# fmbnicola/P3D-RayTracer

Measured on AMD Instinct MI355X. Metric: Mrays/s (primary+secondary), higher is better.
Workload: dtype f32; 1 GPU; balls_low.p3f 1024x1024, Whitted MAX_DEPTH=4, BVH, no AA (BASELINE configs[1]); rays_per_frame=4944908, stack_mode=literal, outputs_per_rank=float RGB + hit ID (16 B/px) + u8 image (3 B/px), all written to HBM, tile_order=cost, frames_in_flight=6, streams=2 bulk (pass 1) + 2 tail (hand-off launches), parallelism=image rows in 8-row stripes, round-robin over 1 GPU(s)

## Files before the change

### p3d-raytracer_amd/__init__.py

```python
import ctypes as C
import os
import subprocess

import numpy as np

HERE = os.path.dirname(os.path.abspath(__file__))
LIB_PATH = os.environ.get("P3D_LIB") or os.path.join(HERE, "libp3d.so")

ACCEL_NONE, ACCEL_GRID, ACCEL_BVH = 0, 1, 2
WHITTED, PATHTRACE = 0, 1
TILE_ORDER_COST, TILE_ORDER_FRAME = 0, 1
STACK_LITERAL, STACK_PER_PIXEL = 0, 1
CHAIN_AUTO, CHAIN_MEGAKERNEL, CHAIN_PER_LEVEL = 0, 1, 2
SAMPLE_JITTER, SAMPLE_TENT = 0, 1
LOAD_LEGACY_F11 = 1
DEBUG_NONE, DEBUG_TEST_INTERSECT, DEBUG_DEPTH_MAP = 0, 1, 2
HANDOFF_COMPACT, HANDOFF_DENSE = 0, 1
UPDATE_REFIT, UPDATE_REBUILD = 0, 1

EXPORTS = [
    "p3d_abi_version", "p3d_last_error", "p3d_device_count", "p3d_config_default",
    "p3d_scene_create", "p3d_scene_create_device_bvh", "p3d_scene_destroy", "p3d_scene_set_skybox", "p3d_render_tile", "p3d_render_tile_device",
    "p3d_scene_status", "p3d_scene_set_tail_stream", "p3d_scene_join", "p3d_object_intercepts", "p3d_object_normal", "p3d_skybox_color",
    "p3d_trace_closest", "p3d_trace_any", "p3d_host_scene_load", "p3d_host_scene_destroy",
# ... 624 lines not shown
                out = acc.render(min(samples_per_pass, acc.total - acc.samples_done), want_rgb8=want_rgb8, stats=stats)
                yield acc.samples_done, out
        finally:
            acc.close()

    def adaptive(self, cfg, rel_error, min_samples=16, tile=None, reserved=(0, 0)):
        return AdaptiveAccumulator(self, cfg, tile or self.full_tile(), rel_error, min_samples, reserved)

    def render_adaptive(self, cfg, samples_per_pass, rel_error, min_samples=16, tile=None, want_rgb8=False, stats=True):
        if samples_per_pass < 1:
            raise ValueError("samples_per_pass must be at least 1")
        ad = self.adaptive(cfg, rel_error, min_samples, tile)
        try:
            while ad.samples_done < ad.total:
                out = ad.render(min(samples_per_pass, ad.total - ad.samples_done), want_rgb8=want_rgb8, stats=stats)
                active = ad.active_pixels
                yield ad.samples_done, active, out
                if active == 0:
                    break
        finally:
            ad.close()

    def status(self):
        return int(self._L.p3d_scene_status(self._h))

    def set_tail_stream(self, stream=None):
        raw = getattr(stream, "cuda_stream", stream)
        _check(self._L.p3d_scene_set_tail_stream(self._h, C.c_void_p(raw) if raw else None))

    def join(self, stream=None, host_wait=False):
        raw = getattr(stream, "cuda_stream", stream)
        _check(self._L.p3d_scene_join(self._h, C.c_void_p(raw) if raw else None, 1 if host_wait else 0))

    def debug_limits(self, trip_bound=0, max_rounds=0, halo_chain=0, leftover_pool=0):
        lim = (C.c_uint32 * 4)(trip_bound, max_rounds, halo_chain, leftover_pool)
        _check(self._L.p3d_debug_scene_limits(self._h, C.cast(lim, C.c_void_p)))

    def render_features(self, cfg, samples=0, tile=None):
        t = tile or self.full_tile()
        nd = np.zeros((t.h, t.w, 4), np.float32)
        ac = np.zeros((t.h, t.w, 4), np.float32)
        _check(self._L.p3d_render_features(self._h, C.byref(cfg), C.byref(t), int(samples), nd.ctypes.data, ac.ctypes.data))
        return nd, ac

    def render_features_device(self, cfg, d_normal_depth, d_albedo_cov, samples=0, tile=None, stream=0):
        raw = getattr(stream, "cuda_stream", stream)
        _check(self._L.p3d_render_features_device(self._h, C.byref(cfg), C.byref(tile or self.full_tile()), int(samples),
                                                  C.c_void_p(d_normal_depth or None), C.c_void_p(d_albedo_cov or None),
                                                  C.c_void_p(raw or None)))

    def render_device(self, cfg, tile, d_rgb=0, d_hit=0, d_rgb8=0, stream=0, stats=None):
        _check(self._L.p3d_render_tile_device(self._h, C.byref(cfg), C.byref(tile), C.c_void_p(d_rgb or None),
                                              C.c_void_p(d_hit or None), C.c_void_p(d_rgb8 or None),
                                              C.c_void_p(stream or None), C.byref(stats) if stats is not None else None))

    def trace_closest(self, accel, origin, direction, want_t=False):
        o = np.ascontiguousarray(origin, np.float32)
        d = np.ascontiguousarray(direction, np.float32)
        n = o.shape[0]
        hit = np.zeros(n, np.int32)
        hp = np.zeros((n, 3), np.float32)
        t = np.zeros(n, np.float32) if want_t else None
        _check(self._L.p3d_trace_closest(self._h, int(accel), n, o.ctypes.data, d.ctypes.data, hit.ctypes.data,
                                         t.ctypes.data if want_t else None, hp.ctypes.data))
        return (hit, hp, t) if want_t else (hit, hp)

    def object_intercepts(self, obj, origin, direction):
        o = np.ascontiguousarray(origin, np.float32)
# ... 336 lines not shown
```

### p3d-raytracer_amd/csrc/capi_common.hpp

```cpp
#pragma once
#include <hip/hip_runtime.h>

#include <algorithm>
#include <cmath>
#include <cstdio>
#include <cstdlib>
#include <cstring>
#include <memory>
#include <string>
#include <type_traits>
#include <vector>

#include "../host/p3d_error.hpp"
#include "kernels.hpp"
#include "lbvh.hpp"
#include "grid_build.hpp"
#include "xform_prims.hpp"
#include "p3d.h"
#include "p3d_debug.h"
#include "wavefront.hpp"
#include "queries.hpp"
#include "pt_kernel.hpp"
#include "adaptive.hpp"
#include "features.hpp"
// ... 46 lines not shown
struct SchedEntry {
  uint32_t accel = 0, aa = 0, spp = 0, pt = 0, tiles_x = 0, tiles_y = 0;
  int32_t max_depth = 0, x0 = 0, y0 = 0, w = 0, h = 0, stripe_h = 0, stripe_stride = 0;
  Scratch cost, sched;
  hipEvent_t ready = nullptr;
  hipStream_t built_on = nullptr;
  uint64_t last_use = 0;
  bool built = false;
  bool same_key(const SchedEntry& o) const {
    return accel == o.accel && aa == o.aa && spp == o.spp && pt == o.pt && tiles_x == o.tiles_x && tiles_y == o.tiles_y && max_depth == o.max_depth && x0 == o.x0 && y0 == o.y0 &&
           w == o.w && h == o.h && stripe_h == o.stripe_h && stripe_stride == o.stripe_stride;
  }
};

}

struct p3d_scene {
  int device = 0;
  std::vector<SchedEntry> sched;
  uint64_t sched_clock = 0;
  float4* d_blob = nullptr;
  uint32_t blob_f4 = 0;
  uint32_t off_nodes = 0, off_bgeom = 0, off_ogeom = 0, off_normals = 0, off_mats = 0, off_lights = 0;
  uint32_t* d_cell_start = nullptr;
  uint32_t* d_cell_items = nullptr;
  uint32_t* d_emitters = nullptr;
  uint32_t* d_sky[6] = {nullptr, nullptr, nullptr, nullptr, nullptr, nullptr};
  bool has_sky = false;
  DevScene dev{};
  bool has_bvh = false, has_grid = false;
  uint32_t bvh_max_depth = 0;
  float device_bvh_ms = 0;
  Scratch levels, spill, deferred, wf_rays, wf_keys, wf_sorted, wf_final, out_rgb, out_hit, out_rgb8, q_in, q_out;
  Scratch ho_where, ho_entries, ho_meta, ho_first, ho_first_sample, ho_touched, ho_lists, ho_check, ho_counters, ho_row_chain, ho_halo_pix, ho_ucount;
  std::vector<int64_t> ho_chain_key;
  bool has_spheres = false;
  uint32_t* d_halo_verdict = nullptr;
  float root_min[3] = {0, 0, 0}, root_max[3] = {0, 0, 0};
  bool zero_weight_reflections = false;
  unsigned long long* d_stats = nullptr;
  uint32_t* d_status = nullptr;
  uint32_t last_status = 0;
  p3d_debug_limits dbg{0, 0, 0, 0};
  hipEvent_t ev0 = nullptr, ev1 = nullptr, ev_mid = nullptr, ev_p1 = nullptr;
  hipStream_t tail_stream = nullptr;
  hipEvent_t ev_tail_go = nullptr, ev_tail_done = nullptr;
  bool tail_pending = false;
  uint64_t cam_gen = 0;
  bool device_bvh = false;
  uint64_t geom_gen = 0;
  std::vector<uint32_t> obj_tm;
  std::vector<float4> create_boxes;
  lbvh::Workspace lbvh_ws;
  bool lbvh_topology = false;
  Scratch upd_stage;
  std::vector<lbvh::UpdateRecord> upd_host;
  Scratch rest;
  Scratch xf_stage;
  std::vector<uint4> xf_host;
  bool uploaded_grid = false;
  uint64_t cell_start_cap = 0, cell_items_cap = 0;
  uint32_t grid_items = 0;
  grid_build::Workspace grid_ws;
};

namespace {

void drop_schedules(p3d_scene* s) {
  for (SchedEntry& e : s->sched)
    if (e.ready) (void)hipEventDestroy(e.ready);
  s->sched.clear();
}

bool camera_usable(const p3d_camera& c) {
  const float f[17] = {c.eye[0], c.eye[1], c.eye[2], c.u[0], c.u[1], c.u[2], c.v[0], c.v[1], c.v[2], c.n[0], c.n[1], c.n[2],
                       c.plane_dist, c.w, c.h, c.focal_ratio, c.aperture};
// ... 46 lines not shown
```

### p3d-raytracer_amd/csrc/capi_debug.hpp

```cpp
#pragma once
#include "capi_common.hpp"

extern "C" {

int p3d_debug_scene_limits(p3d_scene* s, const p3d_debug_limits* limits) {
  static const bool enabled = [] { const char* e = getenv("P3D_TEST_HOOKS"); return e && e[0] == '1' && e[1] == 0; }();
  if (!enabled) return fail(P3D_ERR_UNSUPPORTED, "p3d_debug_scene_limits: test hooks are off (start the process with P3D_TEST_HOOKS=1)");
  if (!s) return fail(P3D_ERR_INVALID, "p3d_debug_scene_limits: null scene");
  s->dbg = limits ? *limits : p3d_debug_limits{0, 0, 0, 0};
  return P3D_OK;
}

#ifdef P3D_PT_PROFILE
int p3d_debug_set_pt_prof(void* device_ptr) {
  unsigned long long* p = static_cast<unsigned long long*>(device_ptr);
  return hipMemcpyToSymbol(HIP_SYMBOL(p3d::g_pt_prof), &p, sizeof(p)) == hipSuccess ? P3D_OK : P3D_ERR_NO_DEVICE;
}
#endif
#ifdef P3D_TIMELINE
int p3d_debug_set_timeline(void* device_ptr) {
  unsigned long long* p = static_cast<unsigned long long*>(device_ptr);
  return hipMemcpyToSymbol(HIP_SYMBOL(p3d::g_timeline), &p, sizeof(p)) == hipSuccess ? P3D_OK : P3D_ERR_NO_DEVICE;
}
int p3d_debug_copy_sched(p3d_scene* s, uint32_t* host_sched, size_t n_sched, uint32_t* host_cost, size_t n_cost) {
  if (s->sched.empty()) return P3D_ERR_INVALID;
  (void)hipDeviceSynchronize();
  if (hipMemcpy(host_sched, s->sched[0].sched.p, n_sched * 4, hipMemcpyDeviceToHost) != hipSuccess) return P3D_ERR_NO_DEVICE;
  return hipMemcpy(host_cost, s->sched[0].cost.p, n_cost * 4, hipMemcpyDeviceToHost) == hipSuccess ? P3D_OK : P3D_ERR_NO_DEVICE;
}
#endif

}
```

### p3d-raytracer_amd/csrc/capi_frame.hpp

```cpp
#pragma once
#include "capi_frame_plan.hpp"

namespace {

constexpr uint32_t kWfHistWords = kWfBins + 32;
#ifndef P3D_REDO_LANES
#define P3D_REDO_LANES 64
#endif
inline uint32_t redo_lanes() {
  static const uint32_t v = [] {
    const char* e = getenv("P3D_REDO_LANES");
    const int n = e ? atoi(e) : P3D_REDO_LANES;
    return (uint32_t)(n >= 1 && n <= 64 ? n : P3D_REDO_LANES);
  }();
  return v;
}
inline uint32_t round1_lanes() {
  static const uint32_t v = [] {
    const char* e = getenv("P3D_ROUND1_LANES");
    const int n = e ? atoi(e) : 64;
    return (uint32_t)(n >= 1 && n <= 64 ? n : 64);
  }();
  return v;
}
// ... 315 lines not shown
    uint64_t pool_entries = H.dense ? (uint64_t)2 * H.cap * H.n_units : s->dbg.leftover_pool ? s->dbg.leftover_pool : std::max<uint64_t>(1u << 16, (uint64_t)kPoolEntriesPerUnit * H.n_units);
    if (!H.dense) pool_entries = std::min<uint64_t>(pool_entries, (uint64_t)2 * H.cap * H.n_units);
    if (pool_entries > 0xffffffffull) return fail(P3D_ERR_CAPACITY, "hit_stack hand-off records exceed 2^32 entries: render the frame in smaller tiles or use P3D_STACK_PER_PIXEL");
    H.pool_cap = (uint32_t)pool_entries;
    if (int rc = s->ho_entries.ensure((size_t)pool_entries * sizeof(uint2))) return rc;
    if (!H.dense)
      if (int rc = s->ho_where.ensure((size_t)2 * H.n_units * sizeof(uint32_t))) return rc;
    if (int rc = s->ho_meta.ensure((size_t)2 * H.n_units * 4)) return rc;
    if (int rc = s->ho_first.ensure((size_t)H.n_units * sizeof(float4))) return rc;
    if (int rc = s->ho_first_sample.ensure(cfg->antialiasing ? (size_t)H.n_units * 4 : 16)) return rc;
    touched_bytes = ((size_t)H.n_units / 32 + 2) * 4;
    if (int rc = s->ho_touched.ensure(touched_bytes)) return rc;
    if (int rc = s->ho_lists.ensure((size_t)4 * H.n_units * sizeof(uint4))) return rc;
    if (!H.dense && !lds_scene)
      if (int rc = s->ho_check.ensure((size_t)H.n_units * sizeof(uint32_t))) return rc;
    counter_words = 32 + (per_level ? ((uint32_t)cfg->max_depth + 1) * (kWfSegments * kWfCounterStride + kWfHistWords) : 0);
    if (int rc = s->ho_counters.ensure((size_t)counter_words * sizeof(uint32_t))) return rc;
    if (per_level) {
      wf_seg_cap = H.n_units / 4 + 4096;
      if (int rc = s->wf_rays.ensure((size_t)kWfSegments * wf_seg_cap * 2 * sizeof(float4))) return rc;
      if (int rc = s->wf_keys.ensure((size_t)kWfSegments * wf_seg_cap * sizeof(uint32_t))) return rc;
      if (int rc = s->wf_sorted.ensure((size_t)H.n_units * 2 * sizeof(float4))) return rc;
      if (int rc = s->wf_final.ensure((size_t)H.n_units * sizeof(float4))) return rc;
    }
    H.entries = (uint2*)s->ho_entries.p;
    H.where = (uint32_t*)s->ho_where.p;
    H.meta = (uint32_t*)s->ho_meta.p;
    H.meta0 = H.meta + H.n_units;
    H.first = (float4*)s->ho_first.p;
    H.first_sample = (uint32_t*)s->ho_first_sample.p;
    H.touched = (uint32_t*)s->ho_touched.p;
    H.row_chain = nullptr;
    H.halo_pix = nullptr;
    if (any_chain) {
      if (int rc = s->ho_row_chain.ensure((size_t)tile->h)) return rc;
      if (int rc = s->ho_halo_pix.ensure((size_t)tile->h * kHaloChain * 4)) return rc;
      H.row_chain = (const uint8_t*)s->ho_row_chain.p;
      H.halo_pix = (const uint32_t*)s->ho_halo_pix.p;
    }
    if (literal && want_counts) {
      if (int rc = s->ho_ucount.ensure((size_t)(kNumStats + kCh0Counters) * H.n_units * sizeof(uint32_t))) return rc;
      H.ucount = (uint32_t*)s->ho_ucount.p;
      H.uch0 = H.ucount + (size_t)kNumStats * H.n_units;
    }
    H.list_cap = H.n_units;
    H.count = want_counts ? 1u : 0u;
    H.max_rounds = std::min<uint32_t>(H.n_units + 2, 4096);
    if (s->dbg.max_rounds) H.max_rounds = s->dbg.max_rounds;
    for (int i = 0; i < 4; ++i) ho_list[i] = (uint4*)s->ho_lists.p + (size_t)i * H.n_units;
    ho_counters = (uint32_t*)s->ho_counters.p;
    H.counters = ho_counters;
    H.pool_top = ho_counters + kHoPoolTop;
    H.check_list = (H.dense || lds_scene) ? nullptr : (uint32_t*)s->ho_check.p;
    H.check_n = ho_counters + kHoCheckN;
    return P3D_OK;
  }

  int halo_memo() {
    const Handoff& H = P.hand;
    if (!plan.literal || !H.halo) return P3D_OK;
    const DevCamera& cam = s->dev.cam;
    halo_blocks = (H.rows * kHaloChain + kBlock - 1) / kBlock;
    const uint32_t max_chain = s->dbg.halo_chain ? std::min<uint32_t>(s->dbg.halo_chain, kHaloChain) : kHaloChain;
    const std::vector<int64_t> key = {tile->x0, tile->y0, tile->w, tile->h, tile->stripe_h, tile->stripe_stride, cam.res_x, cam.res_y,
                                      cfg->antialiasing ? 1 : 0, cfg->antialiasing ? (int64_t)cfg->spp_sqrt : 1, (int64_t)cfg->seed,
                                      cfg->sample_mode, cfg->depth_of_field, cfg->sample_disk, max_chain, (int64_t)(intptr_t)st};
// ... 355 lines not shown
```

### p3d-raytracer_amd/csrc/capi_frame_plan.hpp

```cpp
#pragma once
#include "capi_common.hpp"

namespace {

#ifndef P3D_PT_SUB4_MIN_SPP_SQRT
#define P3D_PT_SUB4_MIN_SPP_SQRT 4
#endif
#ifndef P3D_WHITTED_SUB4_MIN_SPP_SQRT
#define P3D_WHITTED_SUB4_MIN_SPP_SQRT 2
#endif
constexpr uint32_t kWhittedSub4MinSppSqrt = P3D_WHITTED_SUB4_MIN_SPP_SQRT;
constexpr uint32_t kPtSub4MinSppSqrt = P3D_PT_SUB4_MIN_SPP_SQRT;
constexpr uint32_t kLdsSceneLimitBytesPt = 16 * 1024;
constexpr uint32_t kLdsSceneLimitBytes = 26 * 1024;
static_assert(kLdsSceneLimitBytes / 32 < 4096 && kLdsSceneLimitBytesPt / 32 < 4096, "the 6-byte stack entries of LDS-staged scenes keep 12 index bits (device_core.hpp Stack)");
constexpr size_t kLaunchScratchBudget = (size_t)4 << 30;
constexpr uint32_t kMaxLaunchThreads = 1u << 24;

void tile_shape(uint64_t pixels, uint32_t& w, uint32_t& h) {
  static const int forced = [] { const char* e = getenv("P3D_TILE_SHAPE"); return e ? atoi(e) : 0; }();
  int shape = forced;
  if (shape != 88 && shape != 84 && shape != 44) shape = 88;
  w = shape == 44 ? 4 : 8;
  h = shape == 88 ? 8 : 4;
// ... 5 lines not shown
  uint32_t bvh_max_depth, n_lights;
  bool zero_weight_reflections;
};
inline SceneFacts scene_facts(const p3d_scene* s) {
  return SceneFacts{s->off_nodes, s->off_ogeom, s->blob_f4, s->bvh_max_depth, s->dev.n_lights, s->zero_weight_reflections};
}

uint32_t stack_bound(const SceneFacts& s, uint32_t accel, bool whitted) {
  if (accel != P3D_ACCEL_BVH) return 1;
  const uint32_t per = s.bvh_max_depth > 1 ? s.bvh_max_depth - 1 : 1;
  return whitted ? (s.n_lights + 1) * per : per;
}

enum FrameMode { kFrame, kAdaptivePass, kFeatures };

struct FramePlan {
  FrameMode mode;
  bool pt, literal;
  uint32_t bound;
  uint32_t stage_lo, stage_hi;
  bool lds_scene, lds_spill;
  uint32_t window, cap, spill_entries;
  int stack_mode;
  bool sub4, cold_lds;
  uint32_t tpw, tph;
  size_t lds_bytes;
  uint32_t levels, deferred;
  bool per_level;
  int sh, ss;
  uint32_t tiles_x, total_bands, bands_per_launch, xcd_chunk;
  uint32_t halo_blocks_max, adapt_blocks, feat_blocks, max_threads;
  size_t levels_bytes, spill_bytes, deferred_bytes;
  bool sched_ok, repair_tiles;

  uint32_t blocks_for(uint32_t ntiles) const {
    const uint32_t groups = (ntiles + 8 * xcd_chunk - 1) / (8 * xcd_chunk);
    return groups * 8 * xcd_chunk;
  }
};

int plan_frame(const SceneFacts& s, const p3d_config* cfg, const p3d_tile* tile, uint32_t sample_begin, uint32_t sample_end, FrameMode mode,
               uint32_t resident, FramePlan& plan) {
  const bool feat = mode == kFeatures, adapt = mode == kAdaptivePass;
  const uint32_t chain_launch = feat ? (uint32_t)P3D_CHAIN_AUTO : cfg->chain_launch;
  const int sh = tile->stripe_h > 0 ? tile->stripe_h : 1, ss = tile->stripe_h > 0 ? tile->stripe_stride : 1;
  const bool pt = cfg->integrator == P3D_PATHTRACE && cfg->antialiasing;
  const bool literal = !feat && cfg->stack_mode == P3D_STACK_LITERAL && !pt && cfg->accel == P3D_ACCEL_BVH;
  const uint32_t bound = stack_bound(s, cfg->accel, !pt);
  const uint32_t stage_lo = s.off_nodes, stage_hi = (cfg->accel == P3D_ACCEL_BVH && !pt) ? s.off_ogeom : s.blob_f4;
  const size_t stage_bytes = (size_t)(stage_hi - stage_lo) * sizeof(float4);
  const bool lds_scene = stage_bytes <= (pt ? kLdsSceneLimitBytesPt : kLdsSceneLimitBytes) && (bound <= 24 || !pt);
  const bool lds_spill = lds_scene && !pt && (bound > 24 || stage_bytes + (size_t)stack_lds_f4(false, bound) * sizeof(float4) > 20 * 1024);
  uint32_t window = 8;
  if (const char* e = getenv("P3D_LDS_STACK_ENTRIES")) {
    window = 1;
    while (window < (uint32_t)std::max(1, atoi(e)) && window < 1024) window *= 2;
  }
  const bool spilling = cfg->accel == P3D_ACCEL_BVH && !(lds_scene && !lds_spill);
  const uint32_t cap = cfg->accel == P3D_ACCEL_BVH ? (spilling ? window : bound) : 1;
  const uint32_t spill_entries = (spilling && bound > cap) ? bound : 0;
  const uint32_t lds_scene_f4 = lds_scene ? stage_hi - stage_lo : 0;
  const uint32_t launch_samples = sample_end - sample_begin;
  const bool sub4 = !feat && ((pt && launch_samples >= kPtSub4MinSppSqrt * kPtSub4MinSppSqrt) ||
                              (!pt && !literal && !lds_scene && cfg->antialiasing && launch_samples >= kWhittedSub4MinSppSqrt * kWhittedSub4MinSppSqrt));
  const bool cold_lds = !pt && !lds_scene && !cfg->antialiasing;
  uint32_t tpw = sub4 ? 4 : 8, tph = sub4 ? 4 : 8;
// ... 16 lines not shown
  const uint32_t total_bands = ((uint32_t)tile->h + tp - 1) / tp;
  if (tile->stripe_h > 0 && sh % (int)tp == 0 && bands_per_launch >= (uint32_t)sh / tp)
    bands_per_launch = (bands_per_launch / ((uint32_t)sh / tp)) * ((uint32_t)sh / tp);
  bands_per_launch = std::min(bands_per_launch, total_bands);
  if (per_level && bands_per_launch < total_bands) {
    if (chain_launch == P3D_CHAIN_PER_LEVEL) return fail(P3D_ERR_CAPACITY, "chain_launch = PER_LEVEL: tile too large for one launch");
    per_level = false;
    scratch_per_thread += (size_t)levels * sizeof(float4);
    const uint32_t lt = (uint32_t)std::min<size_t>(kMaxLaunchThreads, kLaunchScratchBudget / std::max<size_t>(scratch_per_thread, 1));
    bands_per_launch = std::min(std::max<uint32_t>(1, lt / (tiles_x * kBlock)), total_bands);
    if (tile->stripe_h > 0 && sh % (int)tp == 0 && bands_per_launch >= (uint32_t)sh / tp)
      bands_per_launch = (bands_per_launch / ((uint32_t)sh / tp)) * ((uint32_t)sh / tp);
  }
  plan.mode = mode; plan.pt = pt; plan.literal = literal; plan.bound = bound; plan.stage_lo = stage_lo; plan.stage_hi = stage_hi;
  plan.lds_scene = lds_scene; plan.lds_spill = lds_spill; plan.window = window; plan.cap = cap; plan.spill_entries = spill_entries;
  plan.stack_mode = stack_mode; plan.sub4 = sub4; plan.cold_lds = cold_lds; plan.tpw = tpw; plan.tph = tph; plan.lds_bytes = lds_bytes;
  plan.levels = levels; plan.deferred = deferred; plan.per_level = per_level; plan.sh = sh; plan.ss = ss;
  plan.tiles_x = tiles_x; plan.total_bands = total_bands; plan.bands_per_launch = bands_per_launch;
  plan.xcd_chunk = lds_scene ? 1u : tiles_x;
  plan.sched_ok = cfg->tile_order == P3D_TILE_ORDER_COST && cfg->max_depth > 0;
  const uint32_t halo_blocks_max = plan.halo_blocks_max = literal ? ((uint32_t)tile->h * kHaloChain + kBlock - 1) / kBlock : 0;
  const uint32_t adapt_blocks = plan.adapt_blocks = adapt ? std::max<uint32_t>(1, std::min<uint32_t>(resident, (uint32_t)(((size_t)tile->w * tile->h + (sub4 ? 15 : 63)) / (sub4 ? 16 : 64)))) : 0;
  const uint32_t feat_blocks = plan.feat_blocks = feat ? plan.blocks_for(tiles_x * total_bands) : 0;
  if (feat && (uint64_t)feat_blocks * kBlock * std::max<uint32_t>(spill_entries, 1) > 0xffffffffull)
    return fail(P3D_ERR_CAPACITY, "p3d_render_features: tile too large for one launch over a tree this deep (split the tile)");
  const uint32_t max_threads = plan.max_threads = adapt ? adapt_blocks * kBlock : (feat ? feat_blocks * kBlock : (plan.blocks_for(tiles_x * bands_per_launch) + halo_blocks_max) * kBlock);
  const size_t tile_units = (size_t)tile->h * ((size_t)tile->w + kHaloChain);
  const size_t level_cols = per_level ? std::max<size_t>(tile_units, literal ? (size_t)max_threads : 0) : (size_t)max_threads;
  plan.levels_bytes = std::max<size_t>(16, (size_t)levels * level_cols * sizeof(float4));
  const size_t halo_backing = literal && s.bvh_max_depth > 8 ? (size_t)s.bvh_max_depth * tile->h * kBlock * sizeof(uint2) : 0;
  plan.spill_bytes = std::max<size_t>(16, std::max((size_t)spill_entries * max_threads * sizeof(uint2), halo_backing));
  plan.deferred_bytes = std::max<size_t>(16, (size_t)deferred * max_threads * sizeof(float4));
  plan.repair_tiles = literal && lds_scene && !per_level;
  return P3D_OK;
}

}
```

### p3d-raytracer_amd/csrc/handoff.hpp

```cpp
#pragma once

#include <cstdint>

#include <hip/hip_runtime.h>

namespace p3d {

constexpr uint32_t kHaloChain = 16;
constexpr uint32_t kMetaTouched = 1u << 17;
constexpr uint32_t kNoUnit = 0xffffffffu;

enum HandoffCounter { kHoChecked = 0, kHoRedone, kHoRounds, kHoPoolTop, kHoListA, kHoListB, kHoListC, kHoListD, kHoCheckN, kHoRound0, kHoRound1, kHoNumCounters };
constexpr uint32_t kHoErrLeftoverCap = 1u;
constexpr uint32_t kHoErrNoFixedPoint = 2u;
constexpr uint32_t kHoErrTrips = 4u;
constexpr uint32_t kHoErrList = 8u;
constexpr uint32_t kHoErrHalo = 16u;

struct Handoff {
  uint32_t n_units;
  uint32_t row_units;
  uint32_t halo;
  uint32_t rows;
  uint32_t cap;
  uint32_t persistent;
  uint32_t list_cap;
  uint32_t max_rounds;
  uint32_t round_base;
  uint32_t count;
  uint32_t lanes;
  uint2* entries;
  uint32_t* where;
  uint32_t* pool_top;
  uint32_t* check_list;
  uint32_t* check_n;
  uint32_t pool_cap;
  uint32_t dense;
  uint32_t* meta;
  uint32_t* meta0;
  float4* first;
  uint32_t* first_sample;
  uint32_t* touched;
  const uint8_t* row_chain;
  const uint32_t* halo_pix;
  uint4* list_in;
  uint4* list_out;
  uint32_t* n_in;
  uint32_t* n_out;
  uint32_t* counters;
  uint32_t* ucount;
  uint32_t* uch0;
};
constexpr int kCh0Counters = 5;

__host__ __device__ inline int find_prev_bit(const uint32_t* bits, uint32_t lo, uint32_t i) {
  if (i <= lo) return -1;
  uint32_t w = (i - 1) >> 5;
  const uint32_t wlo = lo >> 5;
  uint32_t word = bits[w] & (0xffffffffu >> (31u - ((i - 1) & 31u)));
  while (true) {
    if (w == wlo) word &= 0xffffffffu << (lo & 31u);
    if (word) return (int)(w * 32u + 31u - (uint32_t)__builtin_clz(word));
    if (w == wlo) return -1;
    --w;
    word = bits[w];
  }
}
__host__ __device__ inline int find_next_bit(const uint32_t* bits, uint32_t i, uint32_t hi) {
  if (i >= hi) return -1;
  uint32_t w = i >> 5;
  const uint32_t whi = (hi - 1) >> 5;
  uint32_t word = bits[w] & (0xffffffffu << (i & 31u));
  while (true) {
    if (w == whi) word &= 0xffffffffu >> (31u - ((hi - 1) & 31u));
    if (word) return (int)(w * 32u + (uint32_t)__builtin_ffs((int)word) - 1u);
    if (w == whi) return -1;
    ++w;
    word = bits[w];
  }
}

__host__ __device__ inline int handoff_pred(const Handoff& H, uint32_t u) {
  if (!H.row_chain) return find_prev_bit(H.touched, 0, u);
  uint32_t row = u / H.row_units, i = u;
  while (true) {
    const uint32_t lo = row * H.row_units;
    const int b = find_prev_bit(H.touched, lo, i);
    if (b >= 0) return b;
    if (H.row_chain[row] || row == 0) return -1;
    i = lo;
    --row;
  }
}
__host__ __device__ inline int handoff_succ(const Handoff& H, uint32_t u) {
  if (!H.row_chain) return find_next_bit(H.touched, u + 1, H.n_units);
  uint32_t row = u / H.row_units, i = u + 1;
  while (true) {
    const uint32_t hi = (row + 1) * H.row_units;
    const int b = find_next_bit(H.touched, i, hi);
    if (b >= 0) return b;
    ++row;
    if (row >= H.rows || H.row_chain[row]) return -1;
    i = hi;
  }
}

__device__ __forceinline__ uint32_t leftover_at(const Handoff& H, uint32_t slot, uint32_t unit) {
  return H.dense ? (slot * H.n_units + unit) * H.cap : H.where[slot * H.n_units + unit];
}
__device__ __forceinline__ uint32_t leftover_alloc(const Handoff& H, uint32_t n, uint32_t slot, uint32_t unit, uint32_t* status, bool announce) {
  if (H.dense) return (slot * H.n_units + unit) * H.cap;
  const uint32_t lane = threadIdx.x & 63u;
  if (announce && H.check_list) {
    const unsigned long long m = __ballot(n != 0);
    uint32_t first = 0;
    if (lane == 63 && m) first = atomicAdd(H.check_n, (uint32_t)__popcll(m));
    first = __shfl(first, 63, 64);
    if (n != 0) H.check_list[first + (uint32_t)__popcll(m & ((1ull << lane) - 1ull))] = unit;
  }
  uint32_t incl = n;
  for (int o = 1; o < 64; o <<= 1) {
    const uint32_t v = __shfl_up(incl, o, 64);
    if ((int)lane >= o) incl += v;
  }
  const uint32_t total = __shfl(incl, 63, 64);
  uint32_t base = 0;
  if (lane == 63 && total) base = atomicAdd(H.pool_top, total);
  base = __shfl(base, 63, 64);
  const uint32_t at = base + incl - n;
  if (n == 0) return kNoUnit;
  if ((unsigned long long)at + n > H.pool_cap) {
    atomicOr(status, kHoErrLeftoverCap);
    return kNoUnit;
  }
  H.where[slot * H.n_units + unit] = at;
  return at;
}

__device__ __forceinline__ bool handoff_touched(const Handoff& H, uint32_t u) { return (H.touched[u >> 5] >> (u & 31u)) & 1u; }
// ... 9 lines not shown
```

### p3d-raytracer_amd/csrc/handoff_kernels.hpp

```cpp

namespace p3d {

struct UnitPlace {
  int c, r, x, y;
  bool halo;
  bool valid;
};
__device__ __forceinline__ UnitPlace no_place() { return UnitPlace{0, 0, 0, 0, false, false}; }
template <class T>
__device__ __forceinline__ T stripe_row(T y0, int r, int sh, int ss) { return y0 + (T)(r / sh) * sh * ss + (r % sh); }
__device__ __forceinline__ int image_row(const RenderParams& P, int r) {
  return stripe_row<int>(P.y0, r, P.stripe_h > 0 ? P.stripe_h : 1, P.stripe_h > 0 ? P.stripe_stride : 1);
}
__device__ __forceinline__ UnitPlace place_of_unit(const RenderParams& P, uint32_t unit) {
  const Handoff& H = P.hand;
  UnitPlace u;
  const uint32_t row = unit / H.row_units, j = unit - row * H.row_units;
  u.r = (int)row - P.row0;
  u.halo = j < H.halo;
  u.valid = true;
  if (u.halo) {
    const uint32_t fp = H.halo_pix[row * H.halo + j];
    u.valid = fp != kNoUnit;
    u.c = 0;
// ... 11 lines not shown
  const uint32_t slot = (blockIdx.x - P.tile_blocks) * kBlock + lane;
  const uint32_t row = slot / kHaloChain, j = slot % kHaloChain;
  if (H.halo == 0 || row >= H.rows || !H.row_chain[row]) return false;
  unit = row * H.row_units + j;
  return H.halo_pix[row * H.halo + j] != kNoUnit;
}
__device__ __forceinline__ bool tile_pixel(const RenderParams& P, uint32_t tx, uint32_t ty, uint32_t tws, uint32_t ths, uint32_t px, int& c, int& r) {
  c = (int)((tx << tws) + (px & ((1u << tws) - 1u)));
  r = (int)((ty << ths) + (px >> tws));
  return px < (1u << (tws + ths)) && c < P.w && r < P.h;
}
__device__ __forceinline__ uint32_t unit_of_pixel(const RenderParams& P, int c, int r) {
  return (uint32_t)(P.row0 + r) * P.hand.row_units + P.hand.halo + (uint32_t)c;
}
__device__ __forceinline__ bool unit_of_lane(const RenderParams& P, bool halo_block, uint32_t tx, uint32_t ty, uint32_t tws, uint32_t ths,
                                             uint32_t lane, uint32_t& unit) {
  if (halo_block) return halo_unit_of_lane(P, lane, unit);
  int c, r;
  const bool in = tile_pixel(P, tx, ty, tws, ths, lane, c, r);
  unit = unit_of_pixel(P, c, r);
  return in;
}
__device__ __forceinline__ uint32_t list_count(const uint32_t* n, uint32_t cap) {
  const uint32_t v = __hip_atomic_load(n, __ATOMIC_RELAXED, __HIP_MEMORY_SCOPE_AGENT);
  return v > cap ? cap : v;
}
__device__ __forceinline__ uint4 list_entry(const uint4* list, uint32_t i) {
  const uint32_t* e = reinterpret_cast<const uint32_t*>(list + i);
  return make_uint4(__hip_atomic_load(e, __ATOMIC_RELAXED, __HIP_MEMORY_SCOPE_AGENT), __hip_atomic_load(e + 1, __ATOMIC_RELAXED, __HIP_MEMORY_SCOPE_AGENT),
                    __hip_atomic_load(e + 2, __ATOMIC_RELAXED, __HIP_MEMORY_SCOPE_AGENT), __hip_atomic_load(e + 3, __ATOMIC_RELAXED, __HIP_MEMORY_SCOPE_AGENT));
}

template <bool SPILL, class CT>
__device__ __forceinline__ void seed_stack(Stack& st, const Handoff& H, uint32_t pred, uint32_t slot_count, CT& ct) {
  stack_clear(st);
  const uint32_t n = slot_count & 0xffffu, slot = slot_count >> 16;
  const uint32_t at = n ? leftover_at(H, slot, pred) : 0u;
  for (uint32_t e = 0; e < n; ++e) {
    const uint2 v = H.entries[at + e];
    push<SPILL>(st, v.x, __uint_as_float(v.y), ct);
  }
}
template <bool STATS>
__device__ __forceinline__ void store_unit_counters(const Handoff& H, uint32_t unit, const Counters<STATS>& ct, const uint32_t* ch0,
                                                    unsigned long long* stats) {
  if (!STATS) return;
  for (int s = 0; s < kNumStats; ++s)
    if (s != kMaxStack) H.ucount[(size_t)s * H.n_units + unit] = ct.get(s);
  for (int k = 0; k < kCh0Counters; ++k) H.uch0[(size_t)k * H.n_units + unit] = ch0[k];
  atomicMax(&stats[kMaxStack], (unsigned long long)ct.get(kMaxStack));
}
template <bool STATS>
__device__ __forceinline__ void replace_ch0_counters(const Handoff& H, uint32_t unit, const Counters<STATS>& cc, unsigned long long* stats) {
  if (!STATS) return;
  for (int k = 0; k < kCh0Counters; ++k) {
    const size_t at = (size_t)k * H.n_units + unit;
    const uint32_t now = cc.get(kNodeTests + k);
    H.ucount[(size_t)(kNodeTests + k) * H.n_units + unit] += now - H.uch0[at];
    H.uch0[at] = now;
  }
  atomicMax(&stats[kMaxStack], (unsigned long long)cc.get(kMaxStack));
}
__global__ void __launch_bounds__(256) ucount_reduce_kernel(const Handoff H, uint32_t w, unsigned long long* stats) {
  const uint32_t i = blockIdx.x * 256 + threadIdx.x;
  const uint32_t n_pix = w * H.rows;
  for (int s = 0; s < kNumStats; ++s) {
    if (s == kMaxStack) continue;
    unsigned long long v = 0;
    for (uint32_t p = i; p < n_pix; p += gridDim.x * 256) {
      const uint32_t unit = (p / w) * H.row_units + H.halo + (p % w);
      v += H.ucount[(size_t)s * H.n_units + unit];
    }
    for (int o = 32; o > 0; o >>= 1) v += __shfl_xor(v, o, 64);
    if ((threadIdx.x & 63) == 0 && v) atomicAdd(&stats[s], v);
// ... 195 lines not shown
    const uint32_t unit = (uint32_t)succ;
    Counters<STATS> ct;
    ct.clear();
    const UnitPlace up = place_of_unit(P, unit);
    const uint32_t slot_count = pm & 0x1ffffu;
    seed_stack<SPILL>(st, H, pred, slot_count, ct);
    if (!first_hit_unchanged<SPILL, !LDS>(P, sc, st, up, unit, P.antialiasing, ct))
      handoff_append(H.list_out, H.n_out, H.list_cap, P.status, make_uint4(unit, pred, slot_count, 0u));
  }
}

template <bool LDS, bool SPILL, bool STATS = false>
__global__ void __launch_bounds__(kBlock) handoff_check_entries_kernel(const RenderParams P) {
  extern __shared__ float4 smem[];
  const Handoff& H = P.hand;
  const uint32_t n = list_count(H.n_in, H.list_cap);
  if ((size_t)blockIdx.x * H.lanes >= n) return;
  const uint32_t lane = threadIdx.x;
  if (H.round_base >= H.max_rounds) {
    if (lane == 0) atomicOr(P.status, kHoErrNoFixedPoint);
    return;
  }
  if (H.count && blockIdx.x == 0 && lane == 0) atomicOr(&H.counters[kHoRound1], 1u);
  DevScene sc = P.sc;
  stage_scene<LDS, false>(sc, P, smem);
  Stack st;
  stack_bind(st, smem, P.lds_scene_f4, lane, P.stack_cap, P.spill, P.level_stride, blockIdx.x * kBlock + lane);
  for (uint32_t chunk = blockIdx.x; (size_t)chunk * H.lanes < n; chunk += gridDim.x) {
    const uint32_t i = chunk * H.lanes + lane;
    if (lane >= H.lanes || i >= n) continue;
    const uint4 e = list_entry(H.list_in, i);
    const UnitPlace up = place_of_unit(P, e.x);
    if (!up.valid) continue;
    if (e.w & 1u) {
      Counters<STATS> ct;
      ct.clear();
      seed_stack<SPILL>(st, H, e.y, e.z, ct);
      if (first_hit_unchanged<SPILL, !LDS>(P, sc, st, up, e.x, P.antialiasing, ct)) continue;
    }
    handoff_append(H.list_out, H.n_out, H.list_cap, P.status, make_uint4(e.x, e.y, e.z, 0u));
  }
}

}
```

### p3d-raytracer_amd/csrc/kernels.hpp

```cpp
#pragma once

#include "device_core.hpp"
#include "handoff.hpp"
#include "p3d.h"

#ifndef P3D_WHITTED_WAVES
#define P3D_WHITTED_WAVES 2
#endif
#ifndef P3D_LIST_WAVES
#define P3D_LIST_WAVES 4
#endif
#ifndef P3D_WHITTED_GLOBAL_WAVES
#define P3D_WHITTED_GLOBAL_WAVES 6
#endif
#ifndef P3D_WHITTED_LDS_WAVES
#define P3D_WHITTED_LDS_WAVES 5
#endif

namespace p3d {

#ifdef P3D_TIMELINE
__device__ unsigned long long* g_timeline = nullptr;
#define P3D_TL_BEGIN() const unsigned long long tl_t0 = wall_clock64();
#define P3D_TL_END()                                                                                  \
// ... 252 lines not shown
  shared.first_hit[px] = -1;
  shared.colour[0][px] = 0.0f; shared.colour[1][px] = 0.0f; shared.colour[2][px] = 0.0f;
  for (int k = 0; k < kPtRing; ++k) shared.tag[k][px] = 0;
}
__device__ __forceinline__ void ring_post(LdsPtPixelShared& shared, uint32_t px, int s, F3 radiance) {
  const int k = s % kPtRing;
  shared.radiance[k][0][px] = radiance.x; shared.radiance[k][1][px] = radiance.y; shared.radiance[k][2][px] = radiance.z;
  shared.tag[k][px] = (uint32_t)s + 1;
}

}

#include "handoff_kernels.hpp"

namespace p3d {

constexpr int whitted_waves(bool AA, bool LDS, int LIT, bool GHOSTS) {
  if (LIT >= 2) return P3D_LIST_WAVES;
  if (AA) return P3D_WHITTED_WAVES;
  if (!LDS) return P3D_WHITTED_GLOBAL_WAVES;
  return (LIT == 1 && GHOSTS) ? P3D_WHITTED_WAVES : P3D_WHITTED_LDS_WAVES;
}
template <int ACCEL, bool LDS, bool STATS, bool AA, bool SPILL = !LDS, int SUB = 1, int LIT = 0, bool GHOSTS = true>
__global__ void __launch_bounds__(kBlock, whitted_waves(AA, LDS, LIT, GHOSTS)) whitted_kernel(const RenderParams P) {
  static_assert(SUB == 1 || AA, "four lanes per pixel need more than one sample per pixel");
  static_assert(LIT == 0 || (ACCEL == P3D_ACCEL_BVH && SUB == 1), "only the BVH has a stack to hand on; one lane per pixel");
  constexpr bool REDO = LIT >= 2;
  constexpr bool GHOST = LIT != 0 && GHOSTS;
  extern __shared__ float4 smem[];
  uint32_t tx = 0, ty = 0;
  const bool halo_block = (LIT == 1 || LIT == 3) && blockIdx.x >= P.tile_blocks;
  if (LIT != 2 && !halo_block && !tile_of_block(P, tx, ty)) return;
  if (LIT == 2 && (size_t)blockIdx.x * P.hand.lanes >= list_count(P.hand.n_in, P.hand.list_cap)) return;
  const uint32_t lane = threadIdx.x;
  const uint32_t tws = SUB == 4 ? 2u : P.tile_w_shift, ths = SUB == 4 ? 2u : P.tile_h_shift;
  uint32_t t_unit = 0, t_pred = 0, t_slot_count = 0;
  bool t_need = false;
  if (LIT == 3) {
    const bool act = unit_of_lane(P, halo_block, tx, ty, tws, ths, lane, t_unit);
    if (act && handoff_touched(P.hand, t_unit)) {
      const int pred = handoff_pred(P.hand, t_unit);
      if (pred >= 0) {
        const uint32_t pm = P.hand.meta0[pred];
        t_need = (pm & 0xffffu) != 0;
        t_pred = (uint32_t)pred;
        t_slot_count = pm & 0x1ffffu;
      }
    }
    if (__ballot(t_need) == 0) return;
  }
  P3D_TL_BEGIN()
  const unsigned long long t_begin = (LIT < 2 && P.tile_cost) ? wall_clock64() : 0;
  DevScene sc = P.sc;
  stage_scene<LDS, ACCEL != P3D_ACCEL_BVH>(sc, P, smem);

  const uint32_t px = SUB == 4 ? lane >> 2 : lane;
  const uint32_t sub = SUB == 4 ? lane & 3u : 0u;
  Counters<STATS> ct;
  if (STATS) reinterpret_cast<Counters<true>&>(ct).clear();
  Stack st;
  stack_bind(st, smem, P.lds_scene_f4, lane, P.stack_cap, P.spill, P.level_stride, blockIdx.x * kBlock + lane);
  const uint32_t gid = blockIdx.x * kBlock + lane;
  constexpr bool COLD = !LDS && !AA;
  constexpr bool VOTE = !LDS;
  ColdState<COLD> cold;
  cold.bind(smem, P.lds_scene_f4 + stack_lds_f4(SPILL, P.stack_cap), lane);
  LdsPtPixelShared& shared = *(LdsPtPixelShared*)(smem + P.lds_scene_f4 + stack_lds_f4(SPILL, P.stack_cap));
  if (SUB == 4 && sub == 0) ring_init(shared, px, P.sample_begin);

  const Handoff& H = P.hand;
  uint4* list_in = H.list_in;
  uint4* list_out = H.list_out;
  uint32_t* n_in_p = H.n_in;
  uint32_t* n_out_p = H.n_out;
  for (uint32_t round = 0;; ++round) {
    uint32_t n_in = 0;
    if (LIT == 2) {
      n_in = list_count(n_in_p, H.list_cap);
      if (n_in == 0) break;
      if (H.round_base + round >= H.max_rounds) {
        if (lane == 0) atomicOr(P.status, kHoErrNoFixedPoint);
        break;
      }
      if (H.count && blockIdx.x == 0 && lane == 0) {
        if (H.round_base + round == 1) atomicOr(&H.counters[kHoRound1], 1u);
        else atomicAdd(&H.counters[kHoRounds], 1u);
      }
    }
    for (uint32_t chunk = blockIdx.x;; chunk += gridDim.x) {
      bool active;
      UnitPlace up = no_place();
      uint32_t unit = 0, pred = 0, pred_slot_count = 0, flags = 0;
      if (LIT == 2) {
        if ((size_t)chunk * H.lanes >= n_in) break;
        const uint32_t i = chunk * H.lanes + lane;
        active = lane < H.lanes && i < n_in;
        if (active) {
          const uint4 e = list_entry(list_in, i);
          unit = e.x; pred = e.y; pred_slot_count = e.z; flags = e.w;
        }
      } else if (LIT == 3) {
        active = t_need;
        unit = t_unit; pred = t_pred; pred_slot_count = t_slot_count; flags = 1u;
      } else if (halo_block) {
        active = halo_unit_of_lane(P, lane, unit);
        up.halo = true;
        if (active) up = place_of_unit(P, unit);
      } else {
        active = tile_pixel(P, tx, ty, tws, ths, px, up.c, up.r);
        up.valid = active;
        up.x = P.x0 + up.c;
        up.y = image_row(P, up.r);
        if (LIT == 1) unit = unit_of_pixel(P, up.c, up.r);
      }
      if (REDO && active) {
        up = place_of_unit(P, unit);
        active = up.valid;
      }

      bool unit_touched = false;
      uint32_t unit_ch0[kCh0Counters] = {0, 0, 0, 0, 0};
      if (STATS && LIT != 0) ct.clear();
      if (REDO && active) {
        seed_stack<SPILL>(st, H, pred, pred_slot_count, ct);
        if (flags & 1u) {
          if (H.count) atomicAdd(&H.counters[kHoChecked], 1u);
          const float4 now = first_closest_hit<SPILL, !LDS>(P, sc, st, up.x, up.y, AA ? H.first_sample[unit] : 0u, ct);
          if (same_first(now, H.first[unit])) {
            active = false;
            replace_ch0_counters<STATS>(H, unit, ct, P.stats);
          } else {
            seed_stack<SPILL>(st, H, pred, pred_slot_count, ct);
// ... 130 lines not shown
            meta = n | kMetaTouched;
            atomicOr(&H.touched[unit >> 5], 1u << (unit & 31u));
          }
          H.meta[unit] = meta;
          H.meta0[unit] = meta;
        }
#endif
        if (LIT != 0 && STATS) {
          if (up.halo) ct.clear();
          store_unit_counters<STATS>(H, unit, ct, unit_ch0, P.stats);
        }
        if (REDO) {
          const uint32_t meta = H.meta[unit];
          const uint32_t cur = (meta >> 16) & 1u, cnt = meta & 0xffffu;
          uint32_t n = (uint32_t)st.sp;
          if (n > H.cap) { atomicOr(P.status, kHoErrLeftoverCap); n = H.cap; }
          bool same = n == cnt;
          const uint32_t old_at = (same && n) ? leftover_at(H, cur, unit) : 0u;
          for (uint32_t e = 0; same && e < n; ++e) {
            const uint2 a = H.entries[old_at + e], b = stack_read<SPILL>(st, (int)e);
            same = a.x == b.x && a.y == b.y;
          }
          if (!same) {
            leave_n = n;
            leave_slot = cur ^ 1u;
            leave_succ = true;
            H.meta[unit] = n | (leave_slot << 16) | kMetaTouched;
          }
        }
      }
#ifdef P3D_ABL_NO_RECORDS
      if (REDO) {
#else
      if (LIT != 0) {
#endif
        const uint32_t at = leftover_alloc(H, leave_n, leave_slot, unit, P.status, LIT == 1 && !LDS);
        if (at != kNoUnit) {
          for (uint32_t e = 0; e < leave_n; ++e) H.entries[at + e] = stack_read<SPILL>(st, (int)e);
        } else if (leave_n) {
          leave_n = 0;
          H.meta[unit] = (leave_slot << 16) | kMetaTouched;
        }
        if (REDO && leave_succ) {
          const int succ = handoff_succ(H, unit);
          if (succ >= 0) handoff_append(list_out, n_out_p, H.list_cap, P.status, make_uint4((uint32_t)succ, unit, (leave_slot << 16) | leave_n, 1u));
        }
      }
      if (LIT != 2) break;
    }
    if (LIT != 2 || !H.persistent) break;
    __threadfence();
    if (lane == 0) __hip_atomic_store(n_in_p, 0u, __ATOMIC_RELAXED, __HIP_MEMORY_SCOPE_AGENT);
    __threadfence();
    uint4* tl = list_in; list_in = list_out; list_out = tl;
    uint32_t* tn = n_in_p; n_in_p = n_out_p; n_out_p = tn;
  }
  if (STATS && LIT == 0) flush_stats<STATS>(ct, P.stats);
  if (LIT < 2 && !halo_block) record_tile_cost(P, tx, ty, t_begin);
  P3D_TL_END()
}

}
```

### p3d-raytracer_amd/csrc/p3d_debug.h

```cpp
#ifndef P3D_DEBUG_H
#define P3D_DEBUG_H
#include "p3d.h"
#ifdef __cplusplus
extern "C" {
#endif
typedef struct p3d_debug_limits {
  uint32_t trip_bound;
  uint32_t max_rounds;
  uint32_t halo_chain;
  uint32_t leftover_pool;
} p3d_debug_limits;
int p3d_debug_scene_limits(p3d_scene* scene, const p3d_debug_limits* limits);
#ifdef __cplusplus
}
#endif
#endif
```

Measured before the change: 47230 Mrays/s.

## Resolve hand-off predecessors from per-tile wave ballot masks instead of global search

Pass 1 now records, per 8x8 tile, 64-bit ballot masks of which pixels touched the hand-off and which left leftover stack entries. The round-0 launch then reads its own tile's and the left neighbour's masks to find each unit's predecessor with bit tricks and skips whole tiles with nothing set, falling back to the global handoff_pred search only when the masks cannot resolve it. Hand-off list entries also carry the leftover offset directly, with the check flag packed into the high bit of the slot word, which saves a leftover_at lookup in the check kernel. The cost is extra mask storage and writes, and correctness now depends on the bit-packing staying consistent between kernels.

```diff
diff --git a/p3d-raytracer_amd/__init__.py b/p3d-raytracer_amd/__init__.py
--- a/p3d-raytracer_amd/__init__.py
+++ b/p3d-raytracer_amd/__init__.py
@@ -680,8 +680,8 @@
         raw = getattr(stream, "cuda_stream", stream)
         _check(self._L.p3d_scene_join(self._h, C.c_void_p(raw) if raw else None, 1 if host_wait else 0))
 
-    def debug_limits(self, trip_bound=0, max_rounds=0, halo_chain=0, leftover_pool=0):
-        lim = (C.c_uint32 * 4)(trip_bound, max_rounds, halo_chain, leftover_pool)
+    def debug_limits(self, trip_bound=0, max_rounds=0, halo_chain=0, leftover_pool=0, no_tile_masks=0):
+        lim = (C.c_uint32 * 5)(trip_bound, max_rounds, halo_chain, leftover_pool, no_tile_masks)
         _check(self._L.p3d_debug_scene_limits(self._h, C.cast(lim, C.c_void_p)))
 
     def render_features(self, cfg, samples=0, tile=None):
diff --git a/p3d-raytracer_amd/csrc/capi_common.hpp b/p3d-raytracer_amd/csrc/capi_common.hpp
--- a/p3d-raytracer_amd/csrc/capi_common.hpp
+++ b/p3d-raytracer_amd/csrc/capi_common.hpp
@@ -102,7 +102,7 @@
   uint32_t bvh_max_depth = 0;
   float device_bvh_ms = 0;
   Scratch levels, spill, deferred, wf_rays, wf_keys, wf_sorted, wf_final, out_rgb, out_hit, out_rgb8, q_in, q_out;
-  Scratch ho_where, ho_entries, ho_meta, ho_first, ho_first_sample, ho_touched, ho_lists, ho_check, ho_counters, ho_row_chain, ho_halo_pix, ho_ucount;
+  Scratch ho_where, ho_entries, ho_meta, ho_first, ho_first_sample, ho_touched, ho_lists, ho_check, ho_counters, ho_row_chain, ho_halo_pix, ho_ucount, ho_tile_masks;
   std::vector<int64_t> ho_chain_key;
   bool has_spheres = false;
   uint32_t* d_halo_verdict = nullptr;
@@ -111,7 +111,7 @@
   unsigned long long* d_stats = nullptr;
   uint32_t* d_status = nullptr;
   uint32_t last_status = 0;
-  p3d_debug_limits dbg{0, 0, 0, 0};
+  p3d_debug_limits dbg{0, 0, 0, 0, 0};
   hipEvent_t ev0 = nullptr, ev1 = nullptr, ev_mid = nullptr, ev_p1 = nullptr;
   hipStream_t tail_stream = nullptr;
   hipEvent_t ev_tail_go = nullptr, ev_tail_done = nullptr;
diff --git a/p3d-raytracer_amd/csrc/capi_debug.hpp b/p3d-raytracer_amd/csrc/capi_debug.hpp
--- a/p3d-raytracer_amd/csrc/capi_debug.hpp
+++ b/p3d-raytracer_amd/csrc/capi_debug.hpp
@@ -7,7 +7,7 @@
   static const bool enabled = [] { const char* e = getenv("P3D_TEST_HOOKS"); return e && e[0] == '1' && e[1] == 0; }();
   if (!enabled) return fail(P3D_ERR_UNSUPPORTED, "p3d_debug_scene_limits: test hooks are off (start the process with P3D_TEST_HOOKS=1)");
   if (!s) return fail(P3D_ERR_INVALID, "p3d_debug_scene_limits: null scene");
-  s->dbg = limits ? *limits : p3d_debug_limits{0, 0, 0, 0};
+  s->dbg = limits ? *limits : p3d_debug_limits{0, 0, 0, 0, 0};
   return P3D_OK;
 }
 
diff --git a/p3d-raytracer_amd/csrc/capi_frame.hpp b/p3d-raytracer_amd/csrc/capi_frame.hpp
--- a/p3d-raytracer_amd/csrc/capi_frame.hpp
+++ b/p3d-raytracer_amd/csrc/capi_frame.hpp
@@ -371,6 +371,13 @@
     H.touched = (uint32_t*)s->ho_touched.p;
     H.row_chain = nullptr;
     H.halo_pix = nullptr;
+    H.tile_touched = nullptr;
+    H.tile_left = nullptr;
+    if (plan.tile_mask_words && !any_chain && !s->dbg.no_tile_masks) {
+      if (int rc = s->ho_tile_masks.ensure(2 * plan.tile_mask_words * sizeof(unsigned long long))) return rc;
+      H.tile_touched = (unsigned long long*)s->ho_tile_masks.p;
+      H.tile_left = H.tile_touched + plan.tile_mask_words;
+    }
     if (any_chain) {
       if (int rc = s->ho_row_chain.ensure((size_t)tile->h)) return rc;
       if (int rc = s->ho_halo_pix.ensure((size_t)tile->h * kHaloChain * 4)) return rc;
diff --git a/p3d-raytracer_amd/csrc/capi_frame_plan.hpp b/p3d-raytracer_amd/csrc/capi_frame_plan.hpp
--- a/p3d-raytracer_amd/csrc/capi_frame_plan.hpp
+++ b/p3d-raytracer_amd/csrc/capi_frame_plan.hpp
@@ -61,6 +61,7 @@
   uint32_t halo_blocks_max, adapt_blocks, feat_blocks, max_threads;
   size_t levels_bytes, spill_bytes, deferred_bytes;
   bool sched_ok, repair_tiles;
+  size_t tile_mask_words;
 
   uint32_t blocks_for(uint32_t ntiles) const {
     const uint32_t groups = (ntiles + 8 * xcd_chunk - 1) / (8 * xcd_chunk);
@@ -143,6 +144,7 @@
   plan.spill_bytes = std::max<size_t>(16, std::max((size_t)spill_entries * max_threads * sizeof(uint2), halo_backing));
   plan.deferred_bytes = std::max<size_t>(16, (size_t)deferred * max_threads * sizeof(float4));
   plan.repair_tiles = literal && lds_scene && !per_level;
+  plan.tile_mask_words = (plan.repair_tiles && tpw == 8 && tph == 8) ? (size_t)tiles_x * total_bands : 0;
   return P3D_OK;
 }
 
diff --git a/p3d-raytracer_amd/csrc/handoff.hpp b/p3d-raytracer_amd/csrc/handoff.hpp
--- a/p3d-raytracer_amd/csrc/handoff.hpp
+++ b/p3d-raytracer_amd/csrc/handoff.hpp
@@ -50,7 +50,10 @@
   uint32_t* counters;
   uint32_t* ucount;
   uint32_t* uch0;
+  unsigned long long* tile_touched;
+  unsigned long long* tile_left;
 };
+constexpr uint32_t kEntryCheck = 1u << 31;
 constexpr int kCh0Counters = 5;
 
 __host__ __device__ inline int find_prev_bit(const uint32_t* bits, uint32_t lo, uint32_t i) {
@@ -105,6 +108,25 @@
   }
 }
 
+struct MaskPred {
+  bool resolved;
+  int pred_lane;
+  bool in_left_tile, left_something;
+};
+__host__ __device__ inline MaskPred handoff_mask_pred(unsigned long long own_touched, unsigned long long own_left, unsigned long long left_touched,
+                                                      unsigned long long left_left, uint32_t lane) {
+  const uint32_t row_shift = lane & 56u, col = lane & 7u;
+  const uint32_t own = (uint32_t)(own_touched >> row_shift) & ((1u << col) - 1u);
+  const uint32_t left = (uint32_t)(left_touched >> row_shift) & 0xffu;
+  MaskPred m{false, -1, false, false};
+  if (own == 0 && left == 0) return m;
+  m.resolved = true;
+  m.in_left_tile = own == 0;
+  m.pred_lane = (int)(row_shift + 31u - (uint32_t)__builtin_clz(own ? own : left));
+  m.left_something = ((m.in_left_tile ? left_left : own_left) >> m.pred_lane) & 1ull;
+  return m;
+}
+
 __device__ __forceinline__ uint32_t leftover_at(const Handoff& H, uint32_t slot, uint32_t unit) {
   return H.dense ? (slot * H.n_units + unit) * H.cap : H.where[slot * H.n_units + unit];
 }
diff --git a/p3d-raytracer_amd/csrc/handoff_kernels.hpp b/p3d-raytracer_amd/csrc/handoff_kernels.hpp
--- a/p3d-raytracer_amd/csrc/handoff_kernels.hpp
+++ b/p3d-raytracer_amd/csrc/handoff_kernels.hpp
@@ -67,14 +67,17 @@
 }
 
 template <bool SPILL, class CT>
-__device__ __forceinline__ void seed_stack(Stack& st, const Handoff& H, uint32_t pred, uint32_t slot_count, CT& ct) {
+__device__ __forceinline__ void seed_stack_at(Stack& st, const Handoff& H, uint32_t at, uint32_t n, CT& ct) {
   stack_clear(st);
-  const uint32_t n = slot_count & 0xffffu, slot = slot_count >> 16;
-  const uint32_t at = n ? leftover_at(H, slot, pred) : 0u;
   for (uint32_t e = 0; e < n; ++e) {
     const uint2 v = H.entries[at + e];
     push<SPILL>(st, v.x, __uint_as_float(v.y), ct);
   }
+}
+template <bool SPILL, class CT>
+__device__ __forceinline__ void seed_stack(Stack& st, const Handoff& H, uint32_t pred, uint32_t slot_count, CT& ct) {
+  const uint32_t n = slot_count & 0xffffu, slot = (slot_count >> 16) & 1u;
+  seed_stack_at<SPILL>(st, H, n ? leftover_at(H, slot, pred) : 0u, n, ct);
 }
 template <bool STATS>
 __device__ __forceinline__ void store_unit_counters(const Handoff& H, uint32_t unit, const Counters<STATS>& ct, const uint32_t* ch0,
@@ -336,14 +339,14 @@
     const uint4 e = list_entry(H.list_in, i);
     const UnitPlace up = place_of_unit(P, e.x);
     if (!up.valid) continue;
-    if (e.w & 1u) {
+    if (e.z & kEntryCheck) {
       Counters<STATS> ct;
       ct.clear();
-      seed_stack<SPILL>(st, H, e.y, e.z, ct);
+      seed_stack_at<SPILL>(st, H, e.w, e.z & 0xffffu, ct);
       if (first_hit_unchanged<SPILL, !LDS>(P, sc, st, up, e.x, P.antialiasing, ct)) continue;
     }
-    handoff_append(H.list_out, H.n_out, H.list_cap, P.status, make_uint4(e.x, e.y, e.z, 0u));
-  }
-}
-
-}
+    handoff_append(H.list_out, H.n_out, H.list_cap, P.status, make_uint4(e.x, e.y, e.z & ~kEntryCheck, e.w));
+  }
+}
+
+}
diff --git a/p3d-raytracer_amd/csrc/kernels.hpp b/p3d-raytracer_amd/csrc/kernels.hpp
--- a/p3d-raytracer_amd/csrc/kernels.hpp
+++ b/p3d-raytracer_amd/csrc/kernels.hpp
@@ -308,13 +308,33 @@
   const bool halo_block = (LIT == 1 || LIT == 3) && blockIdx.x >= P.tile_blocks;
   if (LIT != 2 && !halo_block && !tile_of_block(P, tx, ty)) return;
   if (LIT == 2 && (size_t)blockIdx.x * P.hand.lanes >= list_count(P.hand.n_in, P.hand.list_cap)) return;
+#ifdef P3D_ABL_ROUND0_LEAVE
+  if (LIT == 3) return;
+#endif
   const uint32_t lane = threadIdx.x;
   const uint32_t tws = SUB == 4 ? 2u : P.tile_w_shift, ths = SUB == 4 ? 2u : P.tile_h_shift;
   uint32_t t_unit = 0, t_pred = 0, t_slot_count = 0;
   bool t_need = false;
   if (LIT == 3) {
     const bool act = unit_of_lane(P, halo_block, tx, ty, tws, ths, lane, t_unit);
-    if (act && handoff_touched(P.hand, t_unit)) {
+    const bool masks = P.hand.tile_touched && !halo_block && !P.hand.row_chain && tws == 3 && ths == 3;
+    bool far = !masks && act && handoff_touched(P.hand, t_unit);
+    if (masks) {
+      const uint32_t tile = (((uint32_t)P.row0 >> 3) + ty) * P.tiles_x + tx;
+      const unsigned long long own_t = P.hand.tile_touched[tile], own_l = P.hand.tile_left[tile];
+      const unsigned long long left_t = tx ? P.hand.tile_touched[tile - 1] : 0ull, left_l = tx ? P.hand.tile_left[tile - 1] : 0ull;
+      if ((own_t | own_l) == 0) return;
+      if ((own_t >> lane) & 1ull) {
+        const MaskPred m = handoff_mask_pred(own_t, own_l, left_t, left_l, lane);
+        far = !m.resolved;
+        if (m.left_something) {
+          t_need = true;
+          t_pred = t_unit - (lane & 7u) + ((uint32_t)m.pred_lane & 7u) - (m.in_left_tile ? 8u : 0u);
+          t_slot_count = P.hand.meta0[t_pred] & 0x1ffffu;
+        }
+      }
+    }
+    if (far) {
       const int pred = handoff_pred(P.hand, t_unit);
       if (pred >= 0) {
         const uint32_t pm = P.hand.meta0[pred];
@@ -373,7 +393,7 @@
         active = lane < H.lanes && i < n_in;
         if (active) {
           const uint4 e = list_entry(list_in, i);
-          unit = e.x; pred = e.y; pred_slot_count = e.z; flags = e.w;
+          unit = e.x; pred = e.y; pred_slot_count = e.z & 0x1ffffu; flags = e.z >> 31;
         }
       } else if (LIT == 3) {
         active = t_need;
@@ -570,6 +590,7 @@
 #ifdef P3D_ABL_NO_RECORDS
       if (REDO) {
 #else
+      const unsigned long long wave_touched = LIT == 1 ? __ballot(unit_touched) : 0ull;
       if (LIT != 0) {
 #endif
         const uint32_t at = leftover_alloc(H, leave_n, leave_slot, unit, P.status, LIT == 1 && !LDS);
@@ -579,9 +600,19 @@
           leave_n = 0;
           H.meta[unit] = (leave_slot << 16) | kMetaTouched;
         }
+#ifndef P3D_ABL_NO_RECORDS
+        if (LIT == 1 && H.tile_touched && !halo_block) {
+          const unsigned long long wave_left = __ballot(leave_n != 0);
+          if (lane == 0) {
+            const uint32_t tile = (((uint32_t)P.row0 >> ths) + ty) * P.tiles_x + tx;
+            H.tile_touched[tile] = wave_touched;
+            H.tile_left[tile] = wave_left;
+          }
+        }
+#endif
         if (REDO && leave_succ) {
           const int succ = handoff_succ(H, unit);
-          if (succ >= 0) handoff_append(list_out, n_out_p, H.list_cap, P.status, make_uint4((uint32_t)succ, unit, (leave_slot << 16) | leave_n, 1u));
+          if (succ >= 0) handoff_append(list_out, n_out_p, H.list_cap, P.status, make_uint4((uint32_t)succ, unit, kEntryCheck | (leave_slot << 16) | leave_n, at));
         }
       }
       if (LIT != 2) break;
diff --git a/p3d-raytracer_amd/csrc/p3d_debug.h b/p3d-raytracer_amd/csrc/p3d_debug.h
--- a/p3d-raytracer_amd/csrc/p3d_debug.h
+++ b/p3d-raytracer_amd/csrc/p3d_debug.h
@@ -9,6 +9,7 @@
   uint32_t max_rounds;
   uint32_t halo_chain;
   uint32_t leftover_pool;
+  uint32_t no_tile_masks;
 } p3d_debug_limits;
 int p3d_debug_scene_limits(p3d_scene* scene, const p3d_debug_limits* limits);
 #ifdef __cplusplus
```

Result: faster. 50090 Mrays/s, median of 6 (+6.0%).
